# AssemblyAI-Community/MinImagen

Measured on AMD Instinct MI355X. Metric: denoising-steps/sec (images/sec x T), base 64^2 + SR 64->256 cascade, higher is better.
Workload: dtype f32; 1 GPU; cascade64_256: unet_0 params @64x64 + unet_1 params (lowres_cond) @256x256, T=100/stage, cond_scale=3.0 (2 U-Net evals/step), dynamic thresholding 0.9, fp32 storage / accumulate / softmax / statistics, contractions as 3-term fp16-split (hi*hi + hi*lo + lo*hi) MFMA products; per_gpu_batch=32, global_batch=32, parallelism=dp1

## Files before the change

### include/minimagen_hip.h

```cpp
#ifndef MINIMAGEN_HIP_H
#define MINIMAGEN_HIP_H

#include <stdint.h>

#ifdef __cplusplus
extern "C" {
#endif

#define MI_ABI_VERSION 12

enum mi_status {
    MI_OK = 0,
    MI_ERR_INVALID = -1,
    MI_ERR_LAUNCH = -2,
    MI_ERR_UNSUPPORTED = -3
};

int mi_abi_version(void);
const char* mi_last_error(void);
const char* mi_backend(void);
int mi_struct_size(int which);

typedef struct mi_act {
    const float* data;
// ... 27 lines not shown
    int tile_cfg;
    const void* w_rp;
    const void* res_w_rp;
    int w_rp_exp, res_w_rp_exp;
    float* gn_coef;
    int* gn_exps;
    void* act_prep; long long act_prep_bytes;
} mi_conv_params;
#define MI_CONV_SPLIT16 0x100
#define MI_CONV_SPLIT8  0x800
#define MI_CONV_HALF    0x400
#define MI_CONV_REVERSE 0x200
#define MI_CONV_RP_FIRST 6

int mi_conv_tile_shape(int tile_cfg, int* th, int* tw);
int mi_conv_stripe_rows(const mi_conv_params* p);
int mi_conv_prep_fwd(const mi_conv_params* p, void* stream);
long long mi_conv_prep_bytes(int B, int Cin, int Cres, int H, int W);
int mi_conv_cout_tile(int Cout);
int mi_conv_fwd(const mi_conv_params* p, void* stream);
int mi_gn_coef_fwd(const mi_conv_params* p, void* stream);

typedef struct mi_crossembed_params {
    int B, H, W;
    const float* in0; int C0;
    const float* in1; int C1;
    int in1_batch_mod;
    int in0_batch_mod;
    int n_kernels;
    int ksize[3];
// ... 389 lines not shown
```

### minimagen_amd/_lib.py

```python
from __future__ import annotations

import ctypes as C
import os

import torch

_HERE = os.path.dirname(os.path.abspath(__file__))
DEFAULT_LIB = os.environ.get("MINIMAGEN_HIP_LIB") or os.path.join(_HERE, "libminimagen_hip.so")

c_float_p = C.c_void_p


class MiAct(C.Structure):
    _fields_ = [("data", C.c_void_p), ("C", C.c_int), ("stats", C.c_void_p), ("nt", C.c_int), ("scale", C.c_float), ("bmod", C.c_int),
                ("st", C.c_int)]


class MiConvParams(C.Structure):
    _fields_ = [
        ("B", C.c_int), ("H", C.c_int), ("W", C.c_int),
        ("in0", MiAct), ("in1", MiAct),
        ("Cout", C.c_int), ("ksize", C.c_int), ("stride", C.c_int), ("up2", C.c_int),
        ("w", C.c_void_p), ("bias", C.c_void_p),
        ("gn_groups", C.c_int), ("gn_gamma", C.c_void_p), ("gn_beta", C.c_void_p), ("gn_eps", C.c_float),
# ... 259 lines not shown
    lib.mi_gemm_f32.argtypes = [vp, vp, vp, vp, vp, i32, i32, i32, i32, vp]
    lib.mi_rmsnorm.argtypes = [vp, vp, vp, i32, i32, f32, vp, vp]
    lib.mi_embed_rows.argtypes = [vp, vp, vp, i32, i32, vp]
    lib.mi_embed_rows_sq.argtypes = [vp, vp, vp, vp, i32, i32, i32, vp]
    lib.mi_gemm_rms_f32.argtypes = [vp, vp, vp, vp, vp, i32, i32, i32, i32, vp, i32, f32, vp, vp]
    lib.mi_t5_attention.argtypes = [vp, vp, vp, vp, i32, i32, i32, vp]
    lib.mi_ln_tokens_fwd.argtypes = [vp, i32, i32, vp, vp, vp, vp]
    lib.mi_ln_rows_fwd.argtypes = [vp, vp, vp, vp, i32, i32, f32, vp]
    lib.mi_graph_begin.argtypes = [vp]
    lib.mi_graph_end.argtypes = [vp, C.POINTER(vp)]
    lib.mi_graph_launch.argtypes = [vp, vp]
    lib.mi_graph_destroy.argtypes = [vp]
    lib.mi_conv_tile_shape.argtypes = [i32, C.POINTER(i32), C.POINTER(i32)]
    lib.mi_conv_stripe_rows.argtypes = [vp]
    lib.mi_conv_stripe_rows.restype = i32
    lib.mi_conv_cout_tile.argtypes = [i32]
    lib.mi_init_down_tiles.argtypes = [i32, i32, i32]
    lib.mi_init_down_tiles.restype = i32
    lib.mi_conv_wgrad_workspace.argtypes = [i32, i32, i32]
    lib.mi_conv_wgrad_workspace.restype = C.c_longlong
    lib.mi_crossembed_wgrad_workspace.argtypes = [i32, i32, i32]
    lib.mi_crossembed_wgrad_workspace.restype = C.c_longlong
    lib.mi_chan_stats_fwd.argtypes = [vp, vp, i32, i32, vp]
    lib.mi_layernorm_fwd.argtypes = [vp, vp, vp, vp, vp, i32, i32, C.c_float, vp]
    lib.mi_layernorm_bwd_nwg.argtypes = [i32, i32]
    lib.mi_layernorm_bwd_nwg.restype = i32
    lib.mi_layernorm_bwd.argtypes = [vp, vp, vp, vp, vp, vp, vp, vp, i32, i32, vp]
    lib.mi_pack_conv3_floats.argtypes = [i32, i32, i32, i32, i32]
    lib.mi_pack_conv3_floats.restype = C.c_longlong
    lib.mi_pack_conv3.argtypes = [vp, i32, i32, i32, i32, vp, vp, i32, vp]
# ... 66 lines not shown
```

### minimagen_amd/csrc/conv_stripe.hip

```cpp
#include "rp_common.hip.h"

#ifdef ST_TRACE
__device__ unsigned long long mi_trace_st_buf[1024 * 32];
extern "C" int mi_debug_read_trace_st(void* dst, size_t bytes) { return (int)hipMemcpyFromSymbol(dst, HIP_SYMBOL(mi_trace_st_buf), bytes); }
#define ST_STAMP(k) do { if (lane == 0 && blockIdx.x < 1024) mi_trace_st_buf[blockIdx.x * 32 + (k)] = clock64(); } while (0)
#else
#define ST_STAMP(k) do { } while (0)
#endif

#ifndef ST_ABL
#define ST_ABL 0
#endif
#ifndef ST_BREG
#define ST_BREG 1
#endif
#ifndef ST_HALF_OCTETS
#define ST_HALF_OCTETS 1
#endif
#ifndef ST_NB_HS
#define ST_NB_HS 2
#endif
#ifndef ST_LDG2
#define ST_LDG2 1
#endif
#ifndef ST_LOOKAHEAD
#define ST_LOOKAHEAD 2
#endif
#ifndef ST_RO4
#define ST_RO4 1
#endif
#ifndef ST_LOADER_DELAY
#define ST_LOADER_DELAY 56
#endif

namespace {

template <int W_, int KO_, int NJ_, bool GN_, int OM_, int RO_ = 0>
struct StCfg {
    static constexpr int W = W_, KO = KO_, NJ = NJ_, OM = OM_, RO = RO_;
    static constexpr bool GN = GN_;
    static constexpr bool UP = OM_ == 3, DS = OM_ == 4;
    static constexpr int NTAP = DS ? 4 : 3, NCO = DS ? 16 : 8, OPS = DS ? 1 : 2;
    static constexpr int WS = DS ? 2 * W_ : (UP ? W_ / 2 : W_), RPS = UP ? 1 : 2, NPR = UP ? 3 : 4;
    static constexpr bool HS = W_ < 256 && ST_HALF_OCTETS;
    static constexpr int NCH = HS ? 4 : 8;
    static constexpr int NB = (HS && W_ >= 64) ? ST_NB_HS : 2;
    static constexpr int QPR = WS / 4, UNITS = RPS * QPR * KO * (HS ? 2 : 1), NLWC = (UNITS + 63) / 64;
    static constexpr int LA = W_ <= 128 ? ((NJ_ == 2 && KO_ == 2 && OM_ == 1 && ST_LOOKAHEAD > 1) ? 1 : ST_LOOKAHEAD) : 0;
    static constexpr int LDG = (ST_LDG2 && GN_ && RO_ == 0 && W_ >= 64 && W_ <= 128 && NLWC <= 2) ? 2 : 1;
    static constexpr int NLC = NLWC * LDG;
    static constexpr int UNITS_R = 2 * QPR * RO, NLWR = (UNITS_R + 63) / 64, NLW = NLC + NLWR;
    static constexpr int NG = W_ / 16, NCW = NG >= 4 ? 4 : NG, GPW = NG / NCW;
    static constexpr int NT = (NLW + NCW) * 64;
    static constexpr int PWH = WS / 2 + 2;
    static constexpr int PW = DS ? 2 * PWH : WS + 8, RING = 6, RINGR = 4, PLANE = (KO * RING + RO * RINGR) * PW;
    static constexpr int SR0 = W_ / 8;
    static constexpr int WCH = NTAP * NJ * 128, WTOT = KO * WCH + RO * NJ * 128;
    static constexpr bool BREG = ST_BREG && KO == 1 && NJ == 1 && RO == 0 && !DS && !(LDG == 2 && OM_ == 1);
    static_assert(RO == 0 || (OM_ == 0 && GN_), "a 1x1 residual conv comes with a Block and replaces the identity residual");
    static constexpr int WPE = ((RO > 0 && W_ == 128) || LDG == 2) ? 4 : 1;
    static constexpr bool PHS = HS && 2 * NPR * QPR * KO <= NCW * 64;
    static constexpr int PCH = PHS ? 4 : 8, PU = NPR * QPR * KO * (PHS ? 2 : 1);
    static_assert(PU <= NCW * 64, "the MFMA waves transform the first four rows in one pass");
    static_assert(!DS || (LA > 0 && !GN_ && RO_ == 0 && W_ <= 128), "the stride-2 member is a plain conv, at most 128 output columns");
};

__device__ __forceinline__ bool st_totals_issue(const mi_act& in0, const mi_act& in1, int C0, int Cin, int b, int lane, int nlanes, bool have, mi_stats_regs& r) {
    int TPC = 1;
    while (TPC < 64 && TPC * 2 * Cin <= nlanes) TPC *= 2;
    const int nt_max = (Cin > C0 && in1.nt > in0.nt) ? in1.nt : in0.nt;
    const bool covers = have && TPC * Cin <= nlanes && nt_max <= MI_STATS_K * TPC;
    const int c = lane / TPC, sub = lane % TPC;
    const bool live = covers && c < Cin;
    const bool second = live && c >= C0;
    const int cc = live ? (second ? c - C0 : c) : 0;
// ... 14 lines not shown
    return covers;
}

template <class CFG>
__global__ __launch_bounds__(CFG::NT, CFG::WPE) void conv_stripe_kernel(const mi_conv_params p, const uint4* __restrict__ wrp, const uint4* __restrict__ rwrp, const int nblk) {
    constexpr int W = CFG::W, KO = CFG::KO, NJ = CFG::NJ, QPR = CFG::QPR, UNITS = CFG::UNITS, NLT = CFG::NLW, NLWC = CFG::NLWC, NLC = CFG::NLC, LDG = CFG::LDG, RO = CFG::RO, RINGR = CFG::RINGR;
    constexpr int NCW = CFG::NCW, GPW = CFG::GPW, PW = CFG::PW, RING = CFG::RING, SR0 = CFG::SR0, WCH = CFG::WCH, WTOT = CFG::WTOT, PU = CFG::PU;
    constexpr bool GN = CFG::GN, BREG = CFG::BREG, UP = CFG::UP, DS = CFG::DS;
    constexpr int NTAP = CFG::NTAP, NCO = CFG::NCO, OPS = CFG::OPS, PWH = CFG::PWH;
    constexpr int WS = CFG::WS, RPS = CFG::RPS, NPR = CFG::NPR;
    __shared__ __attribute__((aligned(16))) uint4 actH[CFG::PLANE];
    __shared__ __attribute__((aligned(16))) uint4 actL[CFG::PLANE];
    __shared__ __attribute__((aligned(16))) uint4 wl[BREG ? 1 : WTOT];
    __shared__ __attribute__((aligned(16))) float4 chP[RP_MAXC];
    __shared__ double chS[RP_MAXC], chQ[RP_MAXC], chS2[RO ? RP_MAXC : 1], chQ2[RO ? RP_MAXC : 1];
    __shared__ double red[NCW][2 * NCO * NJ];
    __shared__ int sExp[4];

    const int tid = threadIdx.x, wave = tid >> 6, lane = tid & 63, lq = lane & 15, lg = lane >> 4;
    const int H = p.H, HW = H * W;
    const int Hs = UP ? H / 2 : (DS ? 2 * H : H), HWs = UP ? HW / 4 : (DS ? 4 * HW : HW);
    const int nt = H / SR0;
    const int wgs = nt / nblk;
    int b, sidx;
    if ((p.B & 7) == 0 && !(ST_ABL & 1)) {
        const int L = blockIdx.x;
        int k = L >> 3;
        if (p.tile_cfg & MI_CONV_REVERSE) k = (int)(gridDim.x >> 3) - 1 - k;
        b = (L & 7) + 8 * (k / wgs);
        sidx = k % wgs;
    } else {
// ... 75 lines not shown
        constexpr std::integral_constant<int, 1> B1{};
        {
            mi_stats_regs sr2;
            const int rt = (wave - NLC) * 64 + lane;
            const bool fast2 = st_totals_issue(p.res0, p.res1, Cr0, Cres, b, rt, CFG::NLWR * 64, res_stats, sr2);
            if (fast2) mi_gn_totals_finish(sr2, rt, chS2, chQ2);
            else if (res_stats) mi_gn_channel_totals(p.res0, p.res1, Cr0, Cres, b, rt, CFG::NLWR * 64, chS2, chQ2);
        }
        issue(0, B0);
        issue(1, B1);
        if (have_stats) __syncthreads();
        __syncthreads();
        const float rsc = ldexpf(second ? p.res1.scale : p.res0.scale, sExp[1]);
        uint4* const dstH = &actH[(KO * RING + oct * RINGR + lrow) * PW + 1 + 4 * q];
        uint4* const dstL = &actL[(KO * RING + oct * RINGR + lrow) * PW + 1 + 4 * q];
        auto transform = [&](auto buf_tag) {
            constexpr int buf = decltype(buf_tag)::value;
#pragma unroll
            for (int px = 0; px < 4; ++px) {
                float y[8];
#pragma unroll
                for (int j = 0; j < 8; ++j) y[j] = raw[buf][j][px] * rsc;
                uint4 hv, lv;
                rp_split8(y, hv, lv);
                if (live) { dstH[2 * buf * PW + px] = hv; dstL[2 * buf * PW + px] = lv; }
            }
        };
        transform(B0);
        issue(2, B0);
        __syncthreads();
        for (int it = 0; it < NSTEP; it += 2) {
            transform(B1);
            issue(it + 3, B1);
            __syncthreads();
            transform(B0);
            issue(it + 4, B0);
            __syncthreads();
        }
    } else if (wave < NLT) {
        constexpr int NCH = CFG::NCH, HSM = CFG::HS ? 2 : 1;
        const int grp = LDG > 1 ? wave / NLWC : 0;
        const int u = (wave - grp * NLWC) * 64 + lane;
        const bool live = u < UNITS;
        const int uu = live ? u : 0;
        const int oct = uu / (RPS * QPR * HSM), half = HSM == 2 ? (uu / (RPS * QPR)) & 1 : 0, lrow = RPS == 2 ? (uu / QPR) & 1 : 0, q = uu % QPR;
        const mi_gptr<const float> base = octet_base(oct) + (size_t)(NCH * half) * HWs;
        constexpr int NB = CFG::NB;
        f32x4 raw[NB][NCH];
        bool inimg[NB];
        auto issue = [&](int s, auto buf_tag) {
            constexpr int buf = decltype(buf_tag)::value;
            int y = UP ? ys0 + s + 1 : ys0 + 2 * s + 1 + lrow;
// ... 11 lines not shown
            transform_quad(std::integral_constant<int, NCH>{}, raw[buf], P, inimg[buf], live, oct, half, (UP ? s + 2 : 2 * s + 2 + lrow) % RING, q);
        };
        auto run = [&](auto grp_tag) {
            constexpr int g = decltype(grp_tag)::value;
            if (wave == 0) ST_STAMP(10);
#if ST_LOADER_DELAY && !defined(HIPEMU)
            if constexpr (W <= 128) __builtin_amdgcn_s_sleep(ST_LOADER_DELAY);
#endif
            rp_for_rounds(std::make_integer_sequence<int, NB>{}, [&](auto j) { issue(1 + g + LDG * decltype(j)::value, j); });
            if (wave == 0) ST_STAMP(11);
            if (have_stats) __syncthreads();
            __syncthreads();
            if (wave == 0) ST_STAMP(12);
#pragma unroll
            for (int j = 0; j < NCH; ++j) P[j] = chP[8 * oct + NCH * half + j];
            __syncthreads();
            if (wave == 0) ST_STAMP(14);
            for (int it = 0; it < NSTEP; it += NB * LDG) {
                rp_for_rounds(std::make_integer_sequence<int, NB * LDG>{}, [&](auto jh) {
                    constexpr int j = decltype(jh)::value / LDG, h = decltype(jh)::value % LDG;
                    if constexpr (h == g) {
                        const int t = it + j * LDG + h;
                        if (wave == 0 && t == 2) ST_STAMP(20);
                        transform(t + 1, std::integral_constant<int, j>{});
                        if (wave == 0 && t == 2) ST_STAMP(21);
                        issue(t + 1 + NB * LDG, std::integral_constant<int, j>{});
                        if (wave == 0 && t == 2) ST_STAMP(22);
                    }
                    __syncthreads();
                    if (wave == 0 && it + j * LDG + h == 2) ST_STAMP(23);
// ... 171 lines not shown
        auto issue_res = [&](int it, auto buf_tag) {
            constexpr int buf = decltype(buf_tag)::value;
            if constexpr (idres) {
                const int itc = it < NSTEP ? it : NSTEP - 1;
#pragma unroll
                for (int g = 0; g < GPW; ++g)
#pragma unroll
                    for (int jt = 0; jt < NJ; ++jt) {
                        const int co = 8 * jt + (lq & 7);
                        const int oy = y0 + 2 * itc + dy, ox = 16 * (cw * GPW + g) + 4 * lg;
                        rv[buf][g][jt] = *reinterpret_cast<mi_gptr<const f32x4>>(rbuf + (unsigned)(co * HW + oy * W + ox));
                    }
            }
        };
        float csum[NJ], csq[NJ], cshift[NJ];
        auto compute = [&](int it, auto buf_tag, bool first_of_block) {
            constexpr int buf = decltype(buf_tag)::value;
            f32x4 acc[GPW][NJ];
#pragma unroll
            for (int g = 0; g < GPW; ++g)
#pragma unroll
                for (int jt = 0; jt < NJ; ++jt) acc[g][jt] = (f32x4){0.f, 0.f, 0.f, 0.f};
            if (cw == 0 && it == 2) ST_STAMP(16);
            const int slot = (UP ? it + 1 + ((perm - 1) >> 1) : (DS ? 2 * it + lg : 2 * it + perm)) % RING;
            if constexpr (CFG::LA > 0) {
                constexpr int LA = CFG::LA, NS = NTAP * KO + RO, NBUF = LA + 1;
                rp_f16x8 sah[NBUF][GPW], sal[NBUF][GPW], sbh[NBUF][NJ], sbl[NBUF][NJ];
                const int rslot = RO > 0 ? 2 * (it & 1) + (perm >> 1) : 0;
                auto load = [&](auto st_tag) {
                    constexpr int st = decltype(st_tag)::value, bi = st % NBUF;
                    if constexpr (st < NTAP * KO) {
                        constexpr int o = st / NTAP, t = st % NTAP;
                        if constexpr (!BREG) {
#pragma unroll
                            for (int jt = 0; jt < NJ; ++jt) {
                                sbh[bi][jt] = __builtin_bit_cast(rp_f16x8, wl[o * WCH + (t * NJ + jt) * 128 + lane]);
                                sbl[bi][jt] = __builtin_bit_cast(rp_f16x8, wl[o * WCH + (t * NJ + jt) * 128 + 64 + lane]);
                            }
                        }
#pragma unroll
                        for (int g = 0; g < GPW; ++g) {
                            const int col = 16 * (cw * GPW + g) + lq + t;
                            const int idx = (o * RING + slot) * PW + (DS ? ((t + 1) & 1) * PWH + 16 * (cw * GPW + g) + lq + ((t + 1) >> 1) : (UP ? ((col - 1) >> 1) + 1 : col));
// ... 63 lines not shown
                            const int col = 16 * (cw * GPW + g) + lq + s;
                            const int idx = (o * RING + slot) * PW + (UP ? ((col - 1) >> 1) + 1 : col);
                            const rp_f16x8 ah = __builtin_bit_cast(rp_f16x8, actH[idx]);
                            const rp_f16x8 al = __builtin_bit_cast(rp_f16x8, actL[idx]);
    #pragma unroll
                            for (int jt = 0; jt < NJ; ++jt) {
                                acc[g][jt] = __builtin_amdgcn_mfma_f32_16x16x32_f16(al, bh[jt], acc[g][jt], 0, 0, 0);
                                acc[g][jt] = __builtin_amdgcn_mfma_f32_16x16x32_f16(ah, bl[jt], acc[g][jt], 0, 0, 0);
                            }
    #pragma unroll
                            for (int jt = 0; jt < NJ; ++jt) acc[g][jt] = __builtin_amdgcn_mfma_f32_16x16x32_f16(ah, bh[jt], acc[g][jt], 0, 0, 0);
                        }
                    }
                }
                if constexpr (RO > 0) {
                    const int rslot = 2 * (it & 1) + (perm >> 1);
    #pragma unroll
                    for (int o = 0; o < RO; ++o) {
                        rp_f16x8 bh[NJ], bl[NJ];
    #pragma unroll
                        for (int jt = 0; jt < NJ; ++jt) {
                            bh[jt] = __builtin_bit_cast(rp_f16x8, wl[KO * WCH + (o * NJ + jt) * 128 + lane]);
                            bl[jt] = __builtin_bit_cast(rp_f16x8, wl[KO * WCH + (o * NJ + jt) * 128 + 64 + lane]);
                        }
    #pragma unroll
                        for (int g = 0; g < GPW; ++g) {
                            const int idx = (KO * RING + o * RINGR + rslot) * PW + 16 * (cw * GPW + g) + lq + 1;
                            const rp_f16x8 ah = __builtin_bit_cast(rp_f16x8, actH[idx]);
                            const rp_f16x8 al = __builtin_bit_cast(rp_f16x8, actL[idx]);
    #pragma unroll
                            for (int jt = 0; jt < NJ; ++jt) {
                                acc[g][jt] = __builtin_amdgcn_mfma_f32_16x16x32_f16(al, bh[jt], acc[g][jt], 0, 0, 0);
                                acc[g][jt] = __builtin_amdgcn_mfma_f32_16x16x32_f16(ah, bl[jt], acc[g][jt], 0, 0, 0);
                            }
    #pragma unroll
                            for (int jt = 0; jt < NJ; ++jt) acc[g][jt] = __builtin_amdgcn_mfma_f32_16x16x32_f16(ah, bh[jt], acc[g][jt], 0, 0, 0);
                        }
                    }
                }
            }
#ifdef ST_TRACE
            if (cw == 0 && it == 2) { if (acc[0][0][0] == 123.456f) ST_STAMP(31); ST_STAMP(17); }
#endif
#pragma unroll
            for (int jt = 0; jt < NJ; ++jt) {
                const int co = NCO * jt + (DS ? lq : (lq & 7));
                const float bv = bvv[jt];
                f32x4 yv[GPW];
#pragma unroll
                for (int g = 0; g < GPW; ++g) {
                    f32x4 y;
                    y[0] = fmaf(acc[g][jt][0], unscale, bv); y[1] = fmaf(acc[g][jt][1], unscale, bv);
                    y[2] = fmaf(acc[g][jt][2], unscale, bv); y[3] = fmaf(acc[g][jt][3], unscale, bv);
                    if constexpr (idres) { const f32x4 r = rv[buf][g][jt]; y[0] = fmaf(r[0], rs, y[0]); y[1] = fmaf(r[1], rs, y[1]); y[2] = fmaf(r[2], rs, y[2]); y[3] = fmaf(r[3], rs, y[3]); }
                    yv[g] = y;
                }
                if (first_of_block) {
                    cshift[jt] = __shfl(yv[0][0], DS ? lq : (lq & 7));
                    csum[jt] = 0.f; csq[jt] = 0.f;
                }
                const float cs_ = cshift[jt];
                const bool ok = !MASKC || co < p.Cout;
#pragma unroll
                for (int g = 0; g < GPW; ++g) {
                    const int oy = y0 + OPS * it + dy, ox = 16 * (cw * GPW + g) + 4 * lg;
                    const f32x4 y = yv[g];
                    if constexpr (MASKC) { if (ok) *reinterpret_cast<mi_gptr<f32x4>>(obuf + (unsigned)(co * HW + oy * W + ox)) = y; }
                    else *reinterpret_cast<mi_gptr<f32x4>>(obuf + (unsigned)(co * HW + oy * W + ox)) = y;
                    const float d0 = y[0] - cs_, d1 = y[1] - cs_, d2 = y[2] - cs_, d3 = y[3] - cs_;
                    csum[jt] += ok ? (d0 + d1) + (d2 + d3) : 0.0f;
                    csq[jt] += ok ? fmaf(d0, d0, fmaf(d1, d1, fmaf(d2, d2, d3 * d3))) : 0.0f;
                }
            }
            if (cw == 0 && it == 2) ST_STAMP(18);
        };
        auto flush = [&]() {
            if (!p.out_stats || (ST_ABL & 2)) return;
#pragma unroll
            for (int jt = 0; jt < NJ; ++jt) {
                float s_ = csum[jt], q_ = csq[jt];
                if constexpr (!DS) { s_ += __shfl_xor(s_, 8); q_ += __shfl_xor(q_, 8); }
                s_ += __shfl_xor(s_, 16); q_ += __shfl_xor(q_, 16);
                s_ += __shfl_xor(s_, 32); q_ += __shfl_xor(q_, 32);
                if (lane < NCO) {
                    mi_stat_acc a; a.c = cshift[jt]; a.s = s_; a.q = q_; a.n = GPW * 16 * SR0;
                    mi_stat_finish(a, red[cw][2 * (NCO * jt + lane)], red[cw][2 * (NCO * jt + lane) + 1]);
                }
            }
        };
        auto publish = [&](int blk) {
            if (!p.out_stats || cw != 0 || (ST_ABL & 2)) return;
            if (lane < 2 * NCO * NJ && (lane >> 1) < p.Cout) {
                double v = red[0][lane];
                if constexpr (NCW == 2) v = red[0][lane] + red[1][lane];
                if constexpr (NCW == 4) v = (red[0][lane] + red[1][lane]) + (red[2][lane] + red[3][lane]);
                p.out_stats[((size_t)(b * p.Cout + (lane >> 1)) * nt + blk) * 2 + (lane & 1)] = v;
            }
        };
        issue_res(0, std::integral_constant<int, 0>{});
        __syncthreads();
        if (cw == 0) ST_STAMP(6);
        constexpr int SPB = SR0 / OPS;
#pragma unroll 1
        for (int kb = 0; kb < nblk; ++kb) {
            const int it0 = kb * SPB;
#pragma unroll 1
            for (int i = 0; i < SPB; i += 2) {
                issue_res(it0 + i + 1, std::integral_constant<int, 1>{});
                compute(it0 + i, std::integral_constant<int, 0>{}, i == 0);
                if (cw == 0 && kb == 0 && i == 0) ST_STAMP(7);
                __syncthreads();
                if (cw == 0 && it0 + i == 2) ST_STAMP(19);
                issue_res(it0 + i + 2, std::integral_constant<int, 0>{});
                compute(it0 + i + 1, std::integral_constant<int, 1>{}, false);
                if (i + 2 == SPB) flush();
                __syncthreads();
            }
            if (cw == 0 && kb + 1 == nblk) ST_STAMP(8);
            publish(blk0 + kb);
        }
        if (cw == 0) ST_STAMP(9);
    }
}

template <int W, int KO, int NJ, bool GN, int OM, int RO = 0>
int launch_stripe(const mi_conv_params& p, hipStream_t st) {
    using CFG = StCfg<W, KO, NJ, GN, OM, RO>;
    const int nt = p.H / CFG::SR0;
    int nblk = (p.tile_cfg >> 12) & 0xf;
    if (nblk == 0) nblk = ((W <= 64 || OM == 2) && nt % 2 == 0 && (long long)p.B * (nt / 2) >= 256) ? 2 : 1;
    if (nblk > nt || nt % nblk) nblk = 1;
    hipLaunchKernelGGL(HIP_KERNEL_NAME(conv_stripe_kernel<CFG>), dim3(p.B * (nt / nblk)), dim3(CFG::NT), 0, st, p, (const uint4*)p.w_rp, (const uint4*)p.res_w_rp, nblk);
    return mi_check_launch("conv_stripe_kernel");
}

template <int W>
int launch_stripe_w(const mi_conv_params& p, hipStream_t st, int ko, int nj, bool gn) {
    const int om = p.ksize == 4 ? 4 : (p.up2 ? 3 : (p.Cout < 8 * nj ? 2 : ((p.res0.data && !p.res_w) ? 1 : 0)));
#define ST_BLOCK(KO, NJ) if (gn && ko == KO && nj == NJ) return om == 1 ? launch_stripe<W, KO, NJ, true, 1>(p, st) : launch_stripe<W, KO, NJ, true, 0>(p, st)
#define ST_PLAIN(KO, NJ, OMV) if (!gn && ko == KO && nj == NJ && om == OMV) return launch_stripe<W, KO, NJ, false, OMV>(p, st)
    if constexpr (W == 64 || W == 128) {
        if (gn && ko == 1 && nj == 1 && om == 0 && p.res0.data && p.res_w) return launch_stripe<W, 1, 1, true, 0, 2>(p, st);
    }
    if constexpr (W == 64) {
        if (gn && ko == 2 && nj == 2 && om == 0 && p.res0.data && p.res_w) return launch_stripe<W, 2, 2, true, 0, 4>(p, st);
    }
    if (om <= 1) {
        ST_BLOCK(1, 1);
        if constexpr (W <= 128) { ST_BLOCK(2, 1); }
        if constexpr (W <= 64) { ST_BLOCK(2, 2); ST_BLOCK(4, 2); ST_BLOCK(3, 2); }
    }
    ST_PLAIN(1, 1, 0);
    ST_PLAIN(1, 1, 2);
    if constexpr (W <= 64) { ST_PLAIN(1, 2, 0); }
    if constexpr (W >= 64 && W <= 128) { ST_PLAIN(1, 1, 3); ST_PLAIN(2, 1, 3); }
    if constexpr (W >= 64 && W <= 128) { ST_PLAIN(1, 1, 4); }
#undef ST_BLOCK
#undef ST_PLAIN
    return MI_ERR_UNSUPPORTED;
}
// ... 28 lines not shown
        if (ko_) { *ko_ = ko; *nj_ = nj; }
        return sr0;
    }
    if ((om == 1 && !gn) || (om == 2 && (gn || nj != 1))) return 0;
    const bool common = (ko == 1 && nj == 1) || (p.W <= 128 && ko == 2 && nj == 1 && gn);
    const bool small = p.W <= 64 && ((ko == 2 && nj == 2 && gn) || (ko == 4 && nj == 2 && gn) || (ko == 1 && nj == 2 && !gn) || (ko == 3 && nj == 2 && gn));
    if (!common && !small) return 0;
    if (ko_) { *ko_ = ko; *nj_ = nj; }
    return sr0;
}

}

extern "C" int mi_conv_stripe_rows(const mi_conv_params* pp) { return stripe_block_rows(*pp, nullptr, nullptr); }

int mi_conv_stripe_launch(const mi_conv_params& p, hipStream_t st) {
    int ko = 0, nj = 0;
    if (!stripe_block_rows(p, &ko, &nj)) { mi_set_error("mi_conv_fwd: tile_cfg 12 (full-width stripes) does not take this launch (see mi_conv_stripe_rows)"); return MI_ERR_UNSUPPORTED; }
    const bool gn = p.gn_groups > 0;
    int rc = MI_ERR_UNSUPPORTED;
    switch (p.W) {
        case 32: rc = launch_stripe_w<32>(p, st, ko, nj, gn); break;
        case 64: rc = launch_stripe_w<64>(p, st, ko, nj, gn); break;
        case 128: rc = launch_stripe_w<128>(p, st, ko, nj, gn); break;
        case 256: rc = launch_stripe_w<256>(p, st, ko, nj, gn); break;
    }
    if (rc == MI_ERR_UNSUPPORTED) mi_set_error("mi_conv_fwd: stripe kernel not instantiated for this shape");
    return rc;
}
```

### minimagen_amd/engine.py

```python
from __future__ import annotations

import ctypes as C
import os
from types import SimpleNamespace
from typing import List, Optional

import torch
from torch import nn

from . import _lib as L
from . import packing as P
from .layers import Attention, CrossAttention, EinopsToAndFrom, Identity, Parallel, ResnetBlock, TransformerBlock

MAX_TEXT_LEN = 256
CONV_SPLIT8 = int(os.environ.get("MINIMAGEN_CONV_SPLIT8", "64"))
CONV_RP = int(os.environ.get("MINIMAGEN_CONV_RP", "2"))
CONV_WIDE_GEMM = os.environ.get("MINIMAGEN_CONV_WIDE_GEMM", "1") != "0"
COND_GEMM = int(os.environ.get("MINIMAGEN_COND_GEMM", "2048"))
FLASH_KV_PREP = os.environ.get("MINIMAGEN_FLASH_KV_PREP", "1") != "0"
CE_MFMA = os.environ.get("MINIMAGEN_CE_MFMA", "1") != "0"
ATTN_COND = os.environ.get("MINIMAGEN_ATTN_COND", "1") != "0"
INIT_DOWN = os.environ.get("MINIMAGEN_INIT_DOWN", "1") != "0"
CONV_REVERSE = int(os.environ.get("MINIMAGEN_CONV_REVERSE", "1"))
RP_NTILE = int(os.environ.get("MINIMAGEN_RP_NTILE", "0"))
RP_NTILE_BY = {k: int(os.environ.get("MINIMAGEN_RP_NTILE_" + k, "0")) for k in ("L", "M", "S")}
RP_NTILE_PIPE = {k: int(os.environ.get("MINIMAGEN_RP_NTILE_PIPE_" + k, d)) for k, d in (("L", "0"), ("M", "4"), ("S", "2"))}
CONV_STRIPE = os.environ.get("MINIMAGEN_CONV_STRIPE", "LMS").upper().replace("0", "").replace("1", "LMS")
ST_NBLK = {k: int(os.environ.get("MINIMAGEN_ST_NBLK_" + k, "0")) for k in ("L", "M", "S")}
ST_NBLK_PIPE = {k: int(os.environ.get("MINIMAGEN_ST_NBLK_PIPE_" + k, d)) for k, d in (("L", "0"), ("M", "0"), ("S", "4"))}
WEIGHT_FINGERPRINT = os.environ.get("MINIMAGEN_WEIGHT_FINGERPRINT", "1") != "0"
JT = 17


class Act:
    __slots__ = ("t", "stats", "nt", "C", "H", "W", "batch", "uses", "rev")

    def __init__(self, t, stats, nt, C_, H, W, batch):
        self.t, self.stats, self.nt, self.C, self.H, self.W, self.batch = t, stats, nt, C_, H, W, batch
        self.uses = 0
        self.rev = False

    @property
    def st(self) -> int:
        return 1 if self.t.dtype == torch.bfloat16 else 0
# ... 399 lines not shown
            out.rev = bool(CONV_REVERSE) and batch % 8 == 0 and not in0.rev
            if out.rev:
                p.tile_cfg |= 0x200
            cls = "L" if Ho * Wo > 128 * 128 else ("M" if Ho * Wo > 64 * 64 else "S")
            nt_knob = RP_NTILE_BY[cls] or RP_NTILE
            if not nt_knob and ws.pipelined and RP_NTILE_PIPE[cls] and batch * nt // RP_NTILE_PIPE[cls] >= 256:
                nt_knob = RP_NTILE_PIPE[cls]
            if stripe:
                nt_knob = ST_NBLK[cls]
                if ws.pipelined and ST_NBLK_PIPE[cls] and nt % ST_NBLK_PIPE[cls] == 0 and batch * nt // ST_NBLK_PIPE[cls] >= 128 \
                        and self.unet.lowres_cond:
                    nt_knob = ST_NBLK_PIPE[cls]
                if nt_knob and (nt % nt_knob or nt_knob > 15):
                    nt_knob = 0
            p.tile_cfg |= (nt_knob & 0xf) << 12
            frags = pk.conv_ig if gemm else pk.conv_rp
            frag, p.w_rp_exp = frags[id(wpack)]
            p.w_rp = L.ptr(frag)
            if res is not None and res[2] is not None:
                rfrag, p.res_w_rp_exp = frags[id(res[2])]
                p.res_w_rp = L.ptr(rfrag)
        if wide:
            ws.prog.append((lib.mi_gn_coef_fwd, p, "gn_coef"))
            if gemm:
                ws.ig_convs.append((p, lib.mi_conv_prep_bytes(batch, cin_tot, cres, Ho, Wo)))
                ws.prog.append((lib.mi_conv_prep_fwd, p, "conv_prep"))
        ws.prog.append((lib.mi_conv_fwd, p, "conv"))
        return out

    def _emit_resnet(self, ws, pk, rb: ResnetBlock, in0: Act, in1: Optional[Act]) -> Act:
# ... 534 lines not shown
```

Before: 53240 denoising-steps/s.

## Process two stripe steps per barrier in the stripe conv kernel

Adds a double-step (SPB=2) variant of the full-width stripe conv kernel. Each barrier interval now covers two output row-pairs, using a deeper activation ring, doubled stats reduction buffers and a compute2 path that shares weight fragment loads across both steps. The variant is picked by default for selected 32- and 64-wide block configs, and an env knob can force it on or off. The aim is to halve __syncthreads count and reuse B fragments, at the cost of more LDS, more registers and a tighter lookahead.

```diff
diff --git a/include/minimagen_hip.h b/include/minimagen_hip.h
--- a/include/minimagen_hip.h
+++ b/include/minimagen_hip.h
@@ -65,6 +65,8 @@
 #define MI_CONV_RP_FIRST 6
 
 int mi_conv_tile_shape(int tile_cfg, int* th, int* tw);
+#define MI_CONV_ST_ROWS_SHIFT 16
+int mi_conv_stripe_rows_per_barrier(const mi_conv_params* p);
 int mi_conv_stripe_rows(const mi_conv_params* p);
 int mi_conv_prep_fwd(const mi_conv_params* p, void* stream);
 long long mi_conv_prep_bytes(int B, int Cin, int Cres, int H, int W);
diff --git a/minimagen_amd/_lib.py b/minimagen_amd/_lib.py
--- a/minimagen_amd/_lib.py
+++ b/minimagen_amd/_lib.py
@@ -297,6 +297,8 @@
     lib.mi_conv_tile_shape.argtypes = [i32, C.POINTER(i32), C.POINTER(i32)]
     lib.mi_conv_stripe_rows.argtypes = [vp]
     lib.mi_conv_stripe_rows.restype = i32
+    lib.mi_conv_stripe_rows_per_barrier.argtypes = [vp]
+    lib.mi_conv_stripe_rows_per_barrier.restype = i32
     lib.mi_conv_cout_tile.argtypes = [i32]
     lib.mi_init_down_tiles.argtypes = [i32, i32, i32]
     lib.mi_init_down_tiles.restype = i32
diff --git a/minimagen_amd/csrc/conv_stripe.hip b/minimagen_amd/csrc/conv_stripe.hip
--- a/minimagen_amd/csrc/conv_stripe.hip
+++ b/minimagen_amd/csrc/conv_stripe.hip
@@ -26,6 +26,12 @@
 #ifndef ST_LOOKAHEAD
 #define ST_LOOKAHEAD 2
 #endif
+#ifndef ST_LA2_TIGHT
+#define ST_LA2_TIGHT 1
+#endif
+#ifndef ST_ROWS4
+#define ST_ROWS4 1
+#endif
 #ifndef ST_RO4
 #define ST_RO4 1
 #endif
@@ -35,9 +41,9 @@
 
 namespace {
 
-template <int W_, int KO_, int NJ_, bool GN_, int OM_, int RO_ = 0>
+template <int W_, int KO_, int NJ_, bool GN_, int OM_, int RO_ = 0, int SPB_ = 1>
 struct StCfg {
-    static constexpr int W = W_, KO = KO_, NJ = NJ_, OM = OM_, RO = RO_;
+    static constexpr int W = W_, KO = KO_, NJ = NJ_, OM = OM_, RO = RO_, SPB = SPB_;
     static constexpr bool GN = GN_;
     static constexpr bool UP = OM_ == 3, DS = OM_ == 4;
     static constexpr int NTAP = DS ? 4 : 3, NCO = DS ? 16 : 8, OPS = DS ? 1 : 2;
@@ -53,12 +59,15 @@
     static constexpr int NG = W_ / 16, NCW = NG >= 4 ? 4 : NG, GPW = NG / NCW;
     static constexpr int NT = (NLW + NCW) * 64;
     static constexpr int PWH = WS / 2 + 2;
-    static constexpr int PW = DS ? 2 * PWH : WS + 8, RING = 6, RINGR = 4, PLANE = (KO * RING + RO * RINGR) * PW;
+    static constexpr int PW = DS ? 2 * PWH : WS + 8, RING = SPB_ == 2 ? 10 : 6, RINGR = SPB_ == 2 ? 8 : 4, PLANE = (KO * RING + RO * RINGR) * PW;
     static constexpr int SR0 = W_ / 8;
     static constexpr int WCH = NTAP * NJ * 128, WTOT = KO * WCH + RO * NJ * 128;
     static constexpr bool BREG = ST_BREG && KO == 1 && NJ == 1 && RO == 0 && !DS && !(LDG == 2 && OM_ == 1);
     static_assert(RO == 0 || (OM_ == 0 && GN_), "a 1x1 residual conv comes with a Block and replaces the identity residual");
-    static constexpr int WPE = ((RO > 0 && W_ == 128) || LDG == 2) ? 4 : 1;
+    static constexpr int WPE = (RO > 0 && W_ == 128) ? (SPB_ == 2 ? 2 : 4) : (LDG == 2 ? 4 : 1);
+    static constexpr int LA2 = (WPE == 4 && LA > ST_LA2_TIGHT) ? ST_LA2_TIGHT : LA;
+    static constexpr bool SEQ2 = SPB_ == 2 && W_ == 128 && KO_ == 1 && OM_ == 1 && RO_ == 0;
+    static_assert(SPB_ == 1 || (SPB_ == 2 && LA > 0 && NB == 2 && !UP && !DS && W_ <= 128), "double steps: the plain 3x3 members up to 128 wide");
     static constexpr bool PHS = HS && 2 * NPR * QPR * KO <= NCW * 64;
     static constexpr int PCH = PHS ? 4 : 8, PU = NPR * QPR * KO * (PHS ? 2 : 1);
     static_assert(PU <= NCW * 64, "the MFMA waves transform the first four rows in one pass");
@@ -103,7 +112,7 @@
     __shared__ __attribute__((aligned(16))) uint4 wl[BREG ? 1 : WTOT];
     __shared__ __attribute__((aligned(16))) float4 chP[RP_MAXC];
     __shared__ double chS[RP_MAXC], chQ[RP_MAXC], chS2[RO ? RP_MAXC : 1], chQ2[RO ? RP_MAXC : 1];
-    __shared__ double red[NCW][2 * NCO * NJ];
+    __shared__ double red[CFG::SPB == 2 ? 2 : 1][NCW][2 * NCO * NJ];
     __shared__ int sExp[4];
 
     const int tid = threadIdx.x, wave = tid >> 6, lane = tid & 63, lq = lane & 15, lg = lane >> 4;
@@ -209,8 +218,8 @@
         const float rsc = ldexpf(second ? p.res1.scale : p.res0.scale, sExp[1]);
         uint4* const dstH = &actH[(KO * RING + oct * RINGR + lrow) * PW + 1 + 4 * q];
         uint4* const dstL = &actL[(KO * RING + oct * RINGR + lrow) * PW + 1 + 4 * q];
-        auto transform = [&](auto buf_tag) {
-            constexpr int buf = decltype(buf_tag)::value;
+        auto transform = [&](auto buf_tag, auto half_tag) {
+            constexpr int buf = decltype(buf_tag)::value, roff = (2 * buf + 4 * decltype(half_tag)::value) * PW;
 #pragma unroll
             for (int px = 0; px < 4; ++px) {
                 float y[8];
@@ -218,19 +227,39 @@
                 for (int j = 0; j < 8; ++j) y[j] = raw[buf][j][px] * rsc;
                 uint4 hv, lv;
                 rp_split8(y, hv, lv);
-                if (live) { dstH[2 * buf * PW + px] = hv; dstL[2 * buf * PW + px] = lv; }
+                if (live) { dstH[roff + px] = hv; dstL[roff + px] = lv; }
             }
         };
-        transform(B0);
+        if constexpr (CFG::SPB == 2) {
+            transform(B0, B0);
+            issue(2, B0);
+            transform(B1, B0);
+            issue(3, B1);
+            __syncthreads();
+            for (int T = 0; T < NSTEP / 2; T += 2) {
+                transform(B0, B1);
+                issue(2 * T + 4, B0);
+                transform(B1, B1);
+                issue(2 * T + 5, B1);
+                __syncthreads();
+                transform(B0, B0);
+                issue(2 * T + 6, B0);
+                transform(B1, B0);
+                issue(2 * T + 7, B1);
+                __syncthreads();
+            }
+        } else {
+        transform(B0, B0);
         issue(2, B0);
         __syncthreads();
         for (int it = 0; it < NSTEP; it += 2) {
-            transform(B1);
+            transform(B1, B0);
             issue(it + 3, B1);
             __syncthreads();
-            transform(B0);
+            transform(B0, B0);
             issue(it + 4, B0);
             __syncthreads();
+        }
         }
     } else if (wave < NLT) {
         constexpr int NCH = CFG::NCH, HSM = CFG::HS ? 2 : 1;
@@ -272,6 +301,33 @@
             if (wave == 0) ST_STAMP(12);
 #pragma unroll
             for (int j = 0; j < NCH; ++j) P[j] = chP[8 * oct + NCH * half + j];
+            if constexpr (CFG::SPB == 2) {
+                constexpr std::integral_constant<int, 0> B0{};
+                constexpr std::integral_constant<int, 1> B1{};
+                if constexpr (g == 0) { transform(1, B0); issue(1 + NB * LDG, B0); }
+                __syncthreads();
+                if (wave == 0) ST_STAMP(14);
+                if constexpr (LDG == 1) {
+                    for (int T = 0; T < NSTEP / 2; ++T) {
+                        transform(2 * T + 2, B1);
+                        issue(2 * T + 4, B1);
+                        transform(2 * T + 3, B0);
+                        issue(2 * T + 5, B0);
+                        __syncthreads();
+                    }
+                } else {
+                    static_assert(LDG <= 2, "two loader groups");
+                    for (int T = 0; T < NSTEP / 2; T += 2) {
+                        if constexpr (g == 0) { transform(2 * T + 3, B1); issue(2 * T + 7, B1); }
+                        else { transform(2 * T + 2, B0); issue(2 * T + 6, B0); }
+                        __syncthreads();
+                        if constexpr (g == 0) { transform(2 * T + 5, B0); issue(2 * T + 9, B0); }
+                        else { transform(2 * T + 4, B1); issue(2 * T + 8, B1); }
+                        __syncthreads();
+                    }
+                }
+                return;
+            }
             __syncthreads();
             if (wave == 0) ST_STAMP(14);
             for (int it = 0; it < NSTEP; it += NB * LDG) {
@@ -473,6 +529,38 @@
             }
         };
         float csum[NJ], csq[NJ], cshift[NJ];
+        auto epilogue = [&](int it, const f32x4 (&acc)[GPW][NJ], const f32x4 (&rvb)[idres ? GPW : 1][idres ? NJ : 1], bool first_of_block) {
+#pragma unroll
+            for (int jt = 0; jt < NJ; ++jt) {
+                const int co = NCO * jt + (DS ? lq : (lq & 7));
+                const float bv = bvv[jt];
+                f32x4 yv[GPW];
+#pragma unroll
+                for (int g = 0; g < GPW; ++g) {
+                    f32x4 y;
+                    y[0] = fmaf(acc[g][jt][0], unscale, bv); y[1] = fmaf(acc[g][jt][1], unscale, bv);
+                    y[2] = fmaf(acc[g][jt][2], unscale, bv); y[3] = fmaf(acc[g][jt][3], unscale, bv);
+                    if constexpr (idres) { const f32x4 r = rvb[g][jt]; y[0] = fmaf(r[0], rs, y[0]); y[1] = fmaf(r[1], rs, y[1]); y[2] = fmaf(r[2], rs, y[2]); y[3] = fmaf(r[3], rs, y[3]); }
+                    yv[g] = y;
+                }
+                if (first_of_block) {
+                    cshift[jt] = __shfl(yv[0][0], DS ? lq : (lq & 7));
+                    csum[jt] = 0.f; csq[jt] = 0.f;
+                }
+                const float cs_ = cshift[jt];
+                const bool ok = !MASKC || co < p.Cout;
+#pragma unroll
+                for (int g = 0; g < GPW; ++g) {
+                    const int oy = y0 + OPS * it + dy, ox = 16 * (cw * GPW + g) + 4 * lg;
+                    const f32x4 y = yv[g];
+                    if constexpr (MASKC) { if (ok) *reinterpret_cast<mi_gptr<f32x4>>(obuf + (unsigned)(co * HW + oy * W + ox)) = y; }
+                    else *reinterpret_cast<mi_gptr<f32x4>>(obuf + (unsigned)(co * HW + oy * W + ox)) = y;
+                    const float d0 = y[0] - cs_, d1 = y[1] - cs_, d2 = y[2] - cs_, d3 = y[3] - cs_;
+                    csum[jt] += ok ? (d0 + d1) + (d2 + d3) : 0.0f;
+                    csq[jt] += ok ? fmaf(d0, d0, fmaf(d1, d1, fmaf(d2, d2, d3 * d3))) : 0.0f;
+                }
+            }
+        };
         auto compute = [&](int it, auto buf_tag, bool first_of_block) {
             constexpr int buf = decltype(buf_tag)::value;
             f32x4 acc[GPW][NJ];
@@ -485,7 +573,7 @@
             if constexpr (CFG::LA > 0) {
                 constexpr int LA = CFG::LA, NS = NTAP * KO + RO, NBUF = LA + 1;
                 rp_f16x8 sah[NBUF][GPW], sal[NBUF][GPW], sbh[NBUF][NJ], sbl[NBUF][NJ];
-                const int rslot = RO > 0 ? 2 * (it & 1) + (perm >> 1) : 0;
+                const int rslot = RO > 0 ? 2 * (it & (RINGR / 2 - 1)) + (perm >> 1) : 0;
                 auto load = [&](auto st_tag) {
                     constexpr int st = decltype(st_tag)::value, bi = st % NBUF;
                     if constexpr (st < NTAP * KO) {
@@ -579,7 +667,7 @@
                     }
                 }
                 if constexpr (RO > 0) {
-                    const int rslot = 2 * (it & 1) + (perm >> 1);
+                    const int rslot = 2 * (it & (RINGR / 2 - 1)) + (perm >> 1);
     #pragma unroll
                     for (int o = 0; o < RO; ++o) {
                         rp_f16x8 bh[NJ], bl[NJ];
@@ -607,39 +695,110 @@
 #ifdef ST_TRACE
             if (cw == 0 && it == 2) { if (acc[0][0][0] == 123.456f) ST_STAMP(31); ST_STAMP(17); }
 #endif
-#pragma unroll
-            for (int jt = 0; jt < NJ; ++jt) {
-                const int co = NCO * jt + (DS ? lq : (lq & 7));
-                const float bv = bvv[jt];
-                f32x4 yv[GPW];
-#pragma unroll
-                for (int g = 0; g < GPW; ++g) {
-                    f32x4 y;
-                    y[0] = fmaf(acc[g][jt][0], unscale, bv); y[1] = fmaf(acc[g][jt][1], unscale, bv);
-                    y[2] = fmaf(acc[g][jt][2], unscale, bv); y[3] = fmaf(acc[g][jt][3], unscale, bv);
-                    if constexpr (idres) { const f32x4 r = rv[buf][g][jt]; y[0] = fmaf(r[0], rs, y[0]); y[1] = fmaf(r[1], rs, y[1]); y[2] = fmaf(r[2], rs, y[2]); y[3] = fmaf(r[3], rs, y[3]); }
-                    yv[g] = y;
-                }
-                if (first_of_block) {
-                    cshift[jt] = __shfl(yv[0][0], DS ? lq : (lq & 7));
-                    csum[jt] = 0.f; csq[jt] = 0.f;
-                }
-                const float cs_ = cshift[jt];
-                const bool ok = !MASKC || co < p.Cout;
-#pragma unroll
-                for (int g = 0; g < GPW; ++g) {
-                    const int oy = y0 + OPS * it + dy, ox = 16 * (cw * GPW + g) + 4 * lg;
-                    const f32x4 y = yv[g];
-                    if constexpr (MASKC) { if (ok) *reinterpret_cast<mi_gptr<f32x4>>(obuf + (unsigned)(co * HW + oy * W + ox)) = y; }
-                    else *reinterpret_cast<mi_gptr<f32x4>>(obuf + (unsigned)(co * HW + oy * W + ox)) = y;
-                    const float d0 = y[0] - cs_, d1 = y[1] - cs_, d2 = y[2] - cs_, d3 = y[3] - cs_;
-                    csum[jt] += ok ? (d0 + d1) + (d2 + d3) : 0.0f;
-                    csq[jt] += ok ? fmaf(d0, d0, fmaf(d1, d1, fmaf(d2, d2, d3 * d3))) : 0.0f;
-                }
-            }
+            epilogue(it, acc, rv[buf], first_of_block);
             if (cw == 0 && it == 2) ST_STAMP(18);
         };
-        auto flush = [&]() {
+        auto compute2 = [&](int it, bool first_of_block) {
+            if constexpr (CFG::SEQ2) {
+                compute(it, std::integral_constant<int, 0>{}, first_of_block);
+                compute(it + 1, std::integral_constant<int, 1>{}, false);
+            } else if constexpr (CFG::SPB == 2) {
+                f32x4 acc[2][GPW][NJ];
+#pragma unroll
+                for (int pp = 0; pp < 2; ++pp)
+#pragma unroll
+                    for (int g = 0; g < GPW; ++g)
+#pragma unroll
+                        for (int jt = 0; jt < NJ; ++jt) acc[pp][g][jt] = (f32x4){0.f, 0.f, 0.f, 0.f};
+                if (cw == 0 && it == 2) ST_STAMP(16);
+                constexpr int LA = CFG::LA2, NS = NTAP * KO + RO, NBUF = LA + 1;
+                rp_f16x8 sah[NBUF][2][GPW], sal[NBUF][2][GPW], sbh[NBUF][NJ], sbl[NBUF][NJ];
+                int slot[2], rslot[2];
+#pragma unroll
+                for (int pp = 0; pp < 2; ++pp) {
+                    slot[pp] = (2 * (it + pp) + perm) % RING;
+                    rslot[pp] = RO > 0 ? 2 * ((it + pp) & (RINGR / 2 - 1)) + (perm >> 1) : 0;
+                }
+                auto load = [&](auto st_tag) {
+                    constexpr int st = decltype(st_tag)::value, bi = st % NBUF;
+                    if constexpr (st < NTAP * KO) {
+                        constexpr int o = st / NTAP, t = st % NTAP;
+                        if constexpr (!BREG) {
+#pragma unroll
+                            for (int jt = 0; jt < NJ; ++jt) {
+                                sbh[bi][jt] = __builtin_bit_cast(rp_f16x8, wl[o * WCH + (t * NJ + jt) * 128 + lane]);
+                                sbl[bi][jt] = __builtin_bit_cast(rp_f16x8, wl[o * WCH + (t * NJ + jt) * 128 + 64 + lane]);
+                            }
+                        }
+#pragma unroll
+                        for (int pp = 0; pp < 2; ++pp)
+#pragma unroll
+                            for (int g = 0; g < GPW; ++g) {
+                                const int idx = (o * RING + slot[pp]) * PW + 16 * (cw * GPW + g) + lq + t;
+                                sah[bi][pp][g] = __builtin_bit_cast(rp_f16x8, actH[idx]);
+                                sal[bi][pp][g] = __builtin_bit_cast(rp_f16x8, actL[idx]);
+                            }
+                    } else {
+                        constexpr int o = st - NTAP * KO;
+#pragma unroll
+                        for (int jt = 0; jt < NJ; ++jt) {
+                            sbh[bi][jt] = __builtin_bit_cast(rp_f16x8, wl[KO * WCH + (o * NJ + jt) * 128 + lane]);
+                            sbl[bi][jt] = __builtin_bit_cast(rp_f16x8, wl[KO * WCH + (o * NJ + jt) * 128 + 64 + lane]);
+                        }
+#pragma unroll
+                        for (int pp = 0; pp < 2; ++pp)
+#pragma unroll
+                            for (int g = 0; g < GPW; ++g) {
+                                const int idx = (KO * RING + o * RINGR + rslot[pp]) * PW + 16 * (cw * GPW + g) + lq + 1;
+                                sah[bi][pp][g] = __builtin_bit_cast(rp_f16x8, actH[idx]);
+                                sal[bi][pp][g] = __builtin_bit_cast(rp_f16x8, actL[idx]);
+                            }
+                    }
+                };
+                auto mult = [&](auto st_tag) {
+                    constexpr int st = decltype(st_tag)::value, bi = st % NBUF;
+                    rp_f16x8 bh[NJ], bl[NJ];
+#pragma unroll
+                    for (int jt = 0; jt < NJ; ++jt) {
+                        if constexpr (BREG) { bh[jt] = breg[2 * (st % 3)]; bl[jt] = breg[2 * (st % 3) + 1]; }
+                        else { bh[jt] = sbh[bi][jt]; bl[jt] = sbl[bi][jt]; }
+                    }
+#pragma unroll
+                    for (int pp = 0; pp < 2; ++pp)
+#pragma unroll
+                        for (int g = 0; g < GPW; ++g)
+#pragma unroll
+                            for (int jt = 0; jt < NJ; ++jt) acc[pp][g][jt] = __builtin_amdgcn_mfma_f32_16x16x32_f16(sal[bi][pp][g], bh[jt], acc[pp][g][jt], 0, 0, 0);
+#pragma unroll
+                    for (int pp = 0; pp < 2; ++pp)
+#pragma unroll
+                        for (int g = 0; g < GPW; ++g)
+#pragma unroll
+                            for (int jt = 0; jt < NJ; ++jt) acc[pp][g][jt] = __builtin_amdgcn_mfma_f32_16x16x32_f16(sah[bi][pp][g], bl[jt], acc[pp][g][jt], 0, 0, 0);
+#pragma unroll
+                    for (int pp = 0; pp < 2; ++pp)
+#pragma unroll
+                        for (int g = 0; g < GPW; ++g)
+#pragma unroll
+                            for (int jt = 0; jt < NJ; ++jt) acc[pp][g][jt] = __builtin_amdgcn_mfma_f32_16x16x32_f16(sah[bi][pp][g], bh[jt], acc[pp][g][jt], 0, 0, 0);
+                };
+                rp_for_rounds(std::make_integer_sequence<int, (LA < NS ? LA : NS)>{}, load);
+                rp_for_rounds(std::make_integer_sequence<int, NS>{}, [&](auto st_tag) {
+                    constexpr int st = decltype(st_tag)::value;
+                    if constexpr (st + LA < NS) load(std::integral_constant<int, st + LA>{});
+                    __builtin_amdgcn_sched_barrier(0);
+                    mult(st_tag);
+                    __builtin_amdgcn_sched_barrier(0);
+                });
+#ifdef ST_TRACE
+                if (cw == 0 && it == 2) { if (acc[1][0][0][0] == 123.456f) ST_STAMP(31); ST_STAMP(17); }
+#endif
+                epilogue(it, acc[0], rv[0], first_of_block);
+                epilogue(it + 1, acc[1], rv[1], false);
+                if (cw == 0 && it == 2) ST_STAMP(18);
+            }
+        };
+        auto flush = [&](int rb) {
             if (!p.out_stats || (ST_ABL & 2)) return;
 #pragma unroll
             for (int jt = 0; jt < NJ; ++jt) {
@@ -649,28 +808,51 @@
                 s_ += __shfl_xor(s_, 32); q_ += __shfl_xor(q_, 32);
                 if (lane < NCO) {
                     mi_stat_acc a; a.c = cshift[jt]; a.s = s_; a.q = q_; a.n = GPW * 16 * SR0;
-                    mi_stat_finish(a, red[cw][2 * (NCO * jt + lane)], red[cw][2 * (NCO * jt + lane) + 1]);
+                    mi_stat_finish(a, red[rb][cw][2 * (NCO * jt + lane)], red[rb][cw][2 * (NCO * jt + lane) + 1]);
                 }
             }
         };
-        auto publish = [&](int blk) {
+        auto publish = [&](int blk, int rb) {
             if (!p.out_stats || cw != 0 || (ST_ABL & 2)) return;
             if (lane < 2 * NCO * NJ && (lane >> 1) < p.Cout) {
-                double v = red[0][lane];
-                if constexpr (NCW == 2) v = red[0][lane] + red[1][lane];
-                if constexpr (NCW == 4) v = (red[0][lane] + red[1][lane]) + (red[2][lane] + red[3][lane]);
+                double v = red[rb][0][lane];
+                if constexpr (NCW == 2) v = red[rb][0][lane] + red[rb][1][lane];
+                if constexpr (NCW == 4) v = (red[rb][0][lane] + red[rb][1][lane]) + (red[rb][2][lane] + red[rb][3][lane]);
                 p.out_stats[((size_t)(b * p.Cout + (lane >> 1)) * nt + blk) * 2 + (lane & 1)] = v;
             }
         };
         issue_res(0, std::integral_constant<int, 0>{});
+        constexpr int SPBLK = SR0 / OPS;
+        if constexpr (CFG::SPB == 2) {
+            issue_res(1, std::integral_constant<int, 1>{});
+            __syncthreads();
+            if (cw == 0) ST_STAMP(6);
+#pragma unroll 1
+            for (int kb = 0; kb < nblk; ++kb) {
+                const int it0 = kb * SPBLK;
+#pragma unroll 1
+                for (int i = 0; i < SPBLK; i += 2) {
+                    compute2(it0 + i, i == 0);
+                    if (cw == 0 && kb == 0 && i == 0) ST_STAMP(7);
+                    if (i + 2 == SPBLK) flush(kb & 1);
+                    issue_res(it0 + i + 2, std::integral_constant<int, 0>{});
+                    issue_res(it0 + i + 3, std::integral_constant<int, 1>{});
+                    __syncthreads();
+                    if (cw == 0 && it0 + i == 2) ST_STAMP(19);
+                }
+                if (cw == 0 && kb + 1 == nblk) ST_STAMP(8);
+                publish(blk0 + kb, kb & 1);
+            }
+            if (cw == 0) ST_STAMP(9);
+            return;
+        }
         __syncthreads();
         if (cw == 0) ST_STAMP(6);
-        constexpr int SPB = SR0 / OPS;
 #pragma unroll 1
         for (int kb = 0; kb < nblk; ++kb) {
-            const int it0 = kb * SPB;
+            const int it0 = kb * SPBLK;
 #pragma unroll 1
-            for (int i = 0; i < SPB; i += 2) {
+            for (int i = 0; i < SPBLK; i += 2) {
                 issue_res(it0 + i + 1, std::integral_constant<int, 1>{});
                 compute(it0 + i, std::integral_constant<int, 0>{}, i == 0);
                 if (cw == 0 && kb == 0 && i == 0) ST_STAMP(7);
@@ -678,37 +860,66 @@
                 if (cw == 0 && it0 + i == 2) ST_STAMP(19);
                 issue_res(it0 + i + 2, std::integral_constant<int, 0>{});
                 compute(it0 + i + 1, std::integral_constant<int, 1>{}, false);
-                if (i + 2 == SPB) flush();
+                if (i + 2 == SPBLK) flush(0);
                 __syncthreads();
             }
             if (cw == 0 && kb + 1 == nblk) ST_STAMP(8);
-            publish(blk0 + kb);
+            publish(blk0 + kb, 0);
         }
         if (cw == 0) ST_STAMP(9);
     }
 }
 
+template <int W, int KO, int NJ, bool GN, int OM, int RO>
+constexpr bool st_has_rows4() { return ST_ROWS4 && GN && OM <= 1 && W <= 128 && RO != 4; }
+
+template <int W, int KO, int NJ, bool GN, int OM, int RO>
+constexpr int st_default_spb(int nblk) {
+    if (RO != 0) return 1;
+    if (W == 64) return ((KO == 1 && NJ == 1) || (KO == 2 && NJ == 1 && OM == 0) || (KO == 2 && NJ == 2 && OM == 0)) ? 2 : 1;
+    if (W == 32) return (KO == 2 && NJ == 2) ? 2 : 1;
+    return 1;
+}
+
+template <int W, int KO, int NJ, bool GN, int OM, int RO>
+int st_pick_spb(const mi_conv_params& p, int nblk) {
+    if constexpr (!st_has_rows4<W, KO, NJ, GN, OM, RO>()) return 1;
+    else {
+        const int f = (p.tile_cfg >> MI_CONV_ST_ROWS_SHIFT) & 3;
+        return f == 0 ? st_default_spb<W, KO, NJ, GN, OM, RO>(nblk) : (f == 2 ? 2 : 1);
+    }
+}
+
 template <int W, int KO, int NJ, bool GN, int OM, int RO = 0>
-int launch_stripe(const mi_conv_params& p, hipStream_t st) {
+int launch_stripe(const mi_conv_params& p, hipStream_t st, int* spb_query = nullptr) {
     using CFG = StCfg<W, KO, NJ, GN, OM, RO>;
     const int nt = p.H / CFG::SR0;
     int nblk = (p.tile_cfg >> 12) & 0xf;
     if (nblk == 0) nblk = ((W <= 64 || OM == 2) && nt % 2 == 0 && (long long)p.B * (nt / 2) >= 256) ? 2 : 1;
     if (nblk > nt || nt % nblk) nblk = 1;
+    const int spb = st_pick_spb<W, KO, NJ, GN, OM, RO>(p, nblk);
+    if (spb_query) { *spb_query = spb; return MI_OK; }
+    if constexpr (st_has_rows4<W, KO, NJ, GN, OM, RO>()) {
+        if (spb == 2) {
+            using CFG2 = StCfg<W, KO, NJ, GN, OM, RO, 2>;
+            hipLaunchKernelGGL(HIP_KERNEL_NAME(conv_stripe_kernel<CFG2>), dim3(p.B * (nt / nblk)), dim3(CFG2::NT), 0, st, p, (const uint4*)p.w_rp, (const uint4*)p.res_w_rp, nblk);
+            return mi_check_launch("conv_stripe_kernel");
+        }
+    }
     hipLaunchKernelGGL(HIP_KERNEL_NAME(conv_stripe_kernel<CFG>), dim3(p.B * (nt / nblk)), dim3(CFG::NT), 0, st, p, (const uint4*)p.w_rp, (const uint4*)p.res_w_rp, nblk);
     return mi_check_launch("conv_stripe_kernel");
 }
 
 template <int W>
-int launch_stripe_w(const mi_conv_params& p, hipStream_t st, int ko, int nj, bool gn) {
+int launch_stripe_w(const mi_conv_params& p, hipStream_t st, int ko, int nj, bool gn, int* q = nullptr) {
     const int om = p.ksize == 4 ? 4 : (p.up2 ? 3 : (p.Cout < 8 * nj ? 2 : ((p.res0.data && !p.res_w) ? 1 : 0)));
-#define ST_BLOCK(KO, NJ) if (gn && ko == KO && nj == NJ) return om == 1 ? launch_stripe<W, KO, NJ, true, 1>(p, st) : launch_stripe<W, KO, NJ, true, 0>(p, st)
-#define ST_PLAIN(KO, NJ, OMV) if (!gn && ko == KO && nj == NJ && om == OMV) return launch_stripe<W, KO, NJ, false, OMV>(p, st)
+#define ST_BLOCK(KO, NJ) if (gn && ko == KO && nj == NJ) return om == 1 ? launch_stripe<W, KO, NJ, true, 1>(p, st, q) : launch_stripe<W, KO, NJ, true, 0>(p, st, q)
+#define ST_PLAIN(KO, NJ, OMV) if (!gn && ko == KO && nj == NJ && om == OMV) return launch_stripe<W, KO, NJ, false, OMV>(p, st, q)
     if constexpr (W == 64 || W == 128) {
-        if (gn && ko == 1 && nj == 1 && om == 0 && p.res0.data && p.res_w) return launch_stripe<W, 1, 1, true, 0, 2>(p, st);
+        if (gn && ko == 1 && nj == 1 && om == 0 && p.res0.data && p.res_w) return launch_stripe<W, 1, 1, true, 0, 2>(p, st, q);
     }
     if constexpr (W == 64) {
-        if (gn && ko == 2 && nj == 2 && om == 0 && p.res0.data && p.res_w) return launch_stripe<W, 2, 2, true, 0, 4>(p, st);
+        if (gn && ko == 2 && nj == 2 && om == 0 && p.res0.data && p.res_w) return launch_stripe<W, 2, 2, true, 0, 4>(p, st, q);
     }
     if (om <= 1) {
         ST_BLOCK(1, 1);
@@ -767,8 +978,24 @@
 
 extern "C" int mi_conv_stripe_rows(const mi_conv_params* pp) { return stripe_block_rows(*pp, nullptr, nullptr); }
 
+extern "C" int mi_conv_stripe_rows_per_barrier(const mi_conv_params* pp) {
+    const mi_conv_params& p = *pp;
+    int ko = 0, nj = 0, spb = 0;
+    if (!stripe_block_rows(p, &ko, &nj)) return 0;
+    const bool gn = p.gn_groups > 0;
+    int rc = MI_ERR_UNSUPPORTED;
+    switch (p.W) {
+        case 32: rc = launch_stripe_w<32>(p, nullptr, ko, nj, gn, &spb); break;
+        case 64: rc = launch_stripe_w<64>(p, nullptr, ko, nj, gn, &spb); break;
+        case 128: rc = launch_stripe_w<128>(p, nullptr, ko, nj, gn, &spb); break;
+        case 256: rc = launch_stripe_w<256>(p, nullptr, ko, nj, gn, &spb); break;
+    }
+    return rc == MI_OK ? 2 * spb : 0;
+}
+
 int mi_conv_stripe_launch(const mi_conv_params& p, hipStream_t st) {
     int ko = 0, nj = 0;
+    if (((p.tile_cfg >> MI_CONV_ST_ROWS_SHIFT) & 3) == 3) { mi_set_error("mi_conv_fwd: tile_cfg bits 16..17 (stripe rows per barrier) are 0, 1 or 2"); return MI_ERR_INVALID; }
     if (!stripe_block_rows(p, &ko, &nj)) { mi_set_error("mi_conv_fwd: tile_cfg 12 (full-width stripes) does not take this launch (see mi_conv_stripe_rows)"); return MI_ERR_UNSUPPORTED; }
     const bool gn = p.gn_groups > 0;
     int rc = MI_ERR_UNSUPPORTED;
diff --git a/minimagen_amd/engine.py b/minimagen_amd/engine.py
--- a/minimagen_amd/engine.py
+++ b/minimagen_amd/engine.py
@@ -28,6 +28,7 @@
 CONV_STRIPE = os.environ.get("MINIMAGEN_CONV_STRIPE", "LMS").upper().replace("0", "").replace("1", "LMS")
 ST_NBLK = {k: int(os.environ.get("MINIMAGEN_ST_NBLK_" + k, "0")) for k in ("L", "M", "S")}
 ST_NBLK_PIPE = {k: int(os.environ.get("MINIMAGEN_ST_NBLK_PIPE_" + k, d)) for k, d in (("L", "0"), ("M", "0"), ("S", "4"))}
+ST_ROWS = int(os.environ.get("MINIMAGEN_ST_ROWS", "0")) & 3
 WEIGHT_FINGERPRINT = os.environ.get("MINIMAGEN_WEIGHT_FINGERPRINT", "1") != "0"
 JT = 17
 
@@ -457,6 +458,8 @@
                 if nt_knob and (nt % nt_knob or nt_knob > 15):
                     nt_knob = 0
             p.tile_cfg |= (nt_knob & 0xf) << 12
+            if stripe:
+                p.tile_cfg |= ST_ROWS << 16
             frags = pk.conv_ig if gemm else pk.conv_rp
             frag, p.w_rp_exp = frags[id(wpack)]
             p.w_rp = L.ptr(frag)
```

Measured after the change: 53210 denoising-steps/s. No clear change (-0.1%).
